# iiins0mn1a/shadow-gen

Hardware: AMD Instinct MI355X
Metric: simulated packet events/sec (whole node) at 100k hosts; APSP build time (higher is better)
Workload: dtype u64

## Files before the change

### shadow-gen_amd/csrc/engine.hip

```cpp

#include <hip/hip_runtime.h>

#include <algorithm>
#include <cstring>
#include <string>
#include <tuple>

#include "sgn_internal.h"
#include "sgn_workload.h"

#ifdef SGN_EXP_NODIGEST
#define sgn_drun_add_seq(...) ((void)0)
#define sgn_drun_add_same(...) ((void)0)
#define sgn_drun_flush_seq(...) ((void)0)
#define sgn_drun_flush_same(...) ((void)0)
#define sgn_digest3(h, ...) (h)
#endif

#ifdef SGN_DIAG
#define DG(i) ((void)0)
#define DGT_BEGIN(v) const uint64_t v = __builtin_amdgcn_s_memtime()
#define DGT_END(i, v)                                                                  \
  do {                                                                                 \
    const uint64_t dgt_t = __builtin_amdgcn_s_memtime();                               \
// ... 160 lines not shown
#ifdef SGN_EXP_PLAINCQ
  *p = e;
  return;
#endif
  SGN_GLB char* q = (SGN_GLB char*)p;
  st_wt16(q, e.enqueue_ts, e.eid);
  st_wt16(q + 16, (uint64_t)e.src | ((uint64_t)e.payload << 32), (uint64_t)e.tag | ((uint64_t)e.count << 32));
}

__device__ __forceinline__ void min_nr(SGN_GLB uint64_t* p, uint64_t v) {
  (void)__hip_atomic_fetch_min(p, v, __ATOMIC_RELAXED, __HIP_MEMORY_SCOPE_AGENT);
}

__device__ __forceinline__ void cnt_add(SGN_GLB uint64_t* p, uint64_t v) {
  (void)__hip_atomic_fetch_add(p, v, __ATOMIC_RELAXED, __HIP_MEMORY_SCOPE_AGENT);
}

__device__ __forceinline__ uint64_t div_small(uint64_t a, uint64_t b) {
  if (((a | b) >> 32) == 0) return (uint32_t)a / (uint32_t)b;
  return a / b;
}

__device__ __forceinline__ uint32_t bucket_of(const DevSim& S, uint64_t t) {
  return (uint32_t)S.bw_div.div(t - SIM_START) & (S.NB - 1);
}

__device__ __forceinline__ uint64_t codel_law(uint64_t time, uint64_t count) {
  double sq = count == 0 ? 1.0 : sqrt((double)count);
  double div = 100000000.0 / sq;
  uint64_t inc = (uint64_t)round(div);
  uint64_t orig = time - SIM_START;
  uint64_t adj = orig + inc;
  if (adj < orig || adj > SIMTIME_MAX) adj = SIMTIME_MAX;
  return SIM_START + adj;
}
// ... 617 lines not shown
    else
      fl = (fl & ~(3u << F_RI_STATE_SHIFT)) | (v << F_RI_STATE_SHIFT);
  }

  template <int W>
  __device__ __forceinline__ void forward_later(uint64_t delay) {
    set_relay_state<W>(RELAY_PENDING);
    schedule<W == 0 ? SLOT_RO : SLOT_RI>(now + delay);
  }
  template <int W>
  __device__ __forceinline__ void relay_notify() {
    if (relay_state<W>() == RELAY_IDLE) forward_later<W>(0);
  }

  template <int W>
  __device__ __forceinline__ bool tb_remove(uint64_t dec, uint64_t* dur) {
    DGT_BEGIN(tt);
    const bool ok = tb_remove_<W>(dec, dur);
    DGT_END(DGT_TBRM, tt);
    return ok;
  }
  template <int W>
  __device__ __forceinline__ bool tb_remove_(uint64_t dec, uint64_t* dur) {
    uint64_t& bal = W == 0 ? tbb0 : tbb1;
    uint64_t& last = W == 0 ? tbl0 : tbl1;
    const uint64_t interval = 1000000ULL;
    uint64_t span = now - last;
    if (span >= interval) {
      const uint64_t inc = lr().tbc[W];
      uint64_t nref = span / interval;
      uint64_t ntok = mul_sat(inc, nref, ~0ULL);
      uint64_t b = bal + ntok;
      if (b < bal) b = ~0ULL;
      const uint64_t cap = inc + SGN_CONFIG_MTU;
      bal = b > cap ? cap : b;
      uint64_t adv = mul_sat(interval, nref, SIMTIME_MAX);
      last = emu_sat_add(last, adv);
      span = now - last;
    }
    uint64_t next_refill_span = interval - span;
    if (dec > bal) {
      const uint64_t inc = lr().tbc[W];
      uint64_t req = dec - bal;
      uint64_t n;
      if (((req | inc) >> 32) == 0) {
        const uint32_t r32 = (uint32_t)req, i32 = (uint32_t)inc;
        const uint32_t q = r32 / i32;
        n = q + (r32 - q * i32 ? 1 : 0);
      } else {
        n = req / inc + ((req % inc) ? 1 : 0);
      }
      if (n == 0)
        *dur = 0;
      else if (n == 1)
        *dur = next_refill_span;
      else {
        uint64_t m = mul_sat(interval, n - 1, SIMTIME_MAX);
        uint64_t s = next_refill_span + m;
        if (s < next_refill_span || s > SIMTIME_MAX) s = SIMTIME_MAX;
        *dur = s;
      }
      return false;
    }
    bal -= dec;
    return true;
  }

  template <int K>
  __device__ __forceinline__ void dr_flush_seq() {
#ifndef SGN_EXP_NODIGEST
    const uint32_t n = L->rn[K];
    if (n) L->dig[K] = sgn_digest3(L->dig[K], L->run[K].a, L->run[K].b | ((uint64_t)n << 32), L->run[K].c - n);
    L->rn[K] = 0;
#endif
  }
  template <int K>
  __device__ __forceinline__ void dr_flush_same() {
#ifndef SGN_EXP_NODIGEST
    const uint32_t n = L->rn[K];
    if (n) L->dig[K] = sgn_digest3(L->dig[K], L->run[K].a, L->run[K].b | ((uint64_t)n << 34), L->run[K].c);
// ... 48 lines not shown
      if (I == 3) R->cq_prev = v;
    } else {
      L->cq[I] = v;
    }
  }

  __device__ __forceinline__ SGN_GLB CodelEnt* cq_head_slot() { return S.codel + cq_head; }
  __device__ __forceinline__ SGN_GLB CodelEnt* cq_tail_slot() {
    return S.codel + ((size_t)L->cq_tp * CQ_PAGE + ((cq_head + cq_nr - 1) & (CQ_PAGE - 1)));
  }
  __device__ __forceinline__ uint32_t cq_alloc_page() {
    DGT_BEGIN(ta);
    const uint64_t i = __hip_atomic_fetch_add(&C->pg_alloc, 1ULL, __ATOMIC_RELAXED, __HIP_MEMORY_SCOPE_AGENT);
    cnt_add(ob->pg_allocd, 1);
    if (i >= ob->pg_avail) return NO_HOST;
    const uint32_t pg = ld_dev(&S.cq_free[i % S.cq_pages]);
#ifdef SGN_DIAG
    DGT_WAIT();
    DGT_END(DGT_CQALLOC, ta);
#endif
    return pg;
  }
  __device__ __forceinline__ void cq_free_page(uint32_t pg) {
    DGT_BEGIN(tf);
    const uint64_t j = __hip_atomic_fetch_add(&C->pg_tail, 1ULL, __ATOMIC_RELAXED, __HIP_MEMORY_SCOPE_AGENT);
    st_dev(&S.cq_free[j % S.cq_pages], pg);
    cnt_add(ob->pg_freed, 1);
    DGT_END(DGT_CQFREE, tf);
  }
  __device__ __forceinline__ void cq_pop_head() {
    cq_nr--;
    if (cq_nr == 0) {
      cq_head &= ~(CQ_PAGE - 1);
      L->cq_tp = cq_head / CQ_PAGE;
    } else if (((cq_head + 1) & (CQ_PAGE - 1)) != 0) {
      cq_head++;
    } else {
      const uint32_t pg = cq_head / CQ_PAGE;
      const uint32_t nx = ld_dev(&S.cq_next[pg]);
      cq_free_page(pg);
      cq_head = nx * CQ_PAGE;
// ... 227 lines not shown
        p.payload = ri_pay;
        p.tag = ri_tag;
        p.eid = ri_eid;
      } else {
        if (cq_len > 0) {
          load_head();
          const bool standing = sat_sub(now, L->hd.enqueue_ts) >= CODEL_TARGET;
          const bool ie_due = (fl & F_CODEL_IE) && now >= cqg<0>();
          const bool drop_quiet = (fl & F_CODEL_DROP) && (fl & F_CODEL_DN) && now < cqg<1>();
          if (!standing || !ie_due || drop_quiet) {
            const uint32_t n = L->hd.count;
            const uint64_t wire = (uint64_t)L->hd.payload + sgn_header_bytes(L->hd.tag);
            uint32_t m = n;
            bool blocked = false;
            if (!boot) {
              if (!tb_remove<1>(wire, dur)) {
                m = 0;
                blocked = true;
              } else if (n > 1) {
                const uint64_t more = div_small(tbb1, wire);
                if (more >= n - 1) {
                  tbb1 -= (uint64_t)(n - 1) * wire;
                } else {
                  tbb1 -= more * wire;
                  m = 1 + (uint32_t)more;
                  blocked = true;
                  tb_remove<1>(wire, dur);
                }
              }
            }
            const uint32_t used = m + (blocked ? 1u : 0u);
            const CodelEnt r = L->hd;
            L->hd.eid += used;
            L->hd.count -= used;
            cq_len -= used;
            cq_bytes = sat_sub(cq_bytes, (uint64_t)used * wire);
            if (!standing || cq_bytes <= SGN_CONFIG_MTU) {
              fl &= ~(F_CODEL_IE | F_CODEL_DROP);
            } else if (!ie_due) {
              fl &= ~F_CODEL_DROP;
              if (!(fl & F_CODEL_IE)) {
                fl |= F_CODEL_IE;
                cqs<0>(emu_sat_add(now, CODEL_INTERVAL));
              }
// ... 10 lines not shown
              ri_tag = r.tag;
              ri_eid = r.eid + m;
              set_relay_state<1>(RELAY_IDLE);
              return true;
            }
            continue;
          }
        }
        const bool gotp = codel_pop(&p);
        if (!gotp) {
          set_relay_state<1>(RELAY_IDLE);
          return false;
        }
        DG(DG_FQLOAD);
      }
      if (!boot && !tb_remove<1>((uint64_t)p.payload + sgn_header_bytes(p.tag), dur)) {
        fl |= F_RI_NEXT;
        ri_src = p.src;
        ri_pay = p.payload;
        ri_tag = p.tag;
        ri_eid = p.eid;
        set_relay_state<1>(RELAY_IDLE);
        return true;
      }
      deliver_run(p.src, p.eid, 1, p.payload, p.tag);
    }
  }

  __device__ __forceinline__ void send_batch(uint32_t dst, uint32_t payload, uint32_t tag, uint32_t n,
                                             bool pop = false) {
    DGT_BEGIN(t0);
// ... 252 lines not shown
          st_dev_rec(dstp + pos + m, r);
        else
          st_sys_rec(dstp + pos + m, r);
      } else if (owned)
        place_overflow(S, ob, sidx, pos + m, r);
      else
        spill_run(S, ob, sidx, r);
    }
  }

  __device__ __forceinline__ void forward_out_step() {
    DGT_BEGIN(tf0);
    const bool boot = now < S.boot_end;
    uint64_t dur = 0;
    bool blocked = false;
    if (fl & F_RO_NEXT) {
      fl &= ~F_RO_NEXT;
      const bool is_local = ro_dst == gid;
      if (!boot && !is_local && !tb_remove<0>((uint64_t)ro_pay + sgn_header_bytes(ro_tag), &dur)) {
        fl |= F_RO_NEXT;
        blocked = true;
      } else {
        Pkt p;
        p.src = gid;
        p.dst_ip = my_ip;
        p.payload = ro_pay;
        p.tag = ro_tag;
        p.eid = 0;
        if (is_local)
          deliver_local(p);
        else
          send_batch(ro_dst, ro_pay, ro_tag, 1);
      }
    } else if (fq_len > 0) {
      const FifoEnt e = fifo_head();
      const bool rr = S.qdisc_rr && fq_len > 1;
      const uint32_t run = (e.count == 1 || rr) ? 1u : e.count - 1;
      const uint32_t payload = e.count == 1 ? (e.pay >> 16) : (e.pay & 0xFFFFu);
      const uint64_t wire = (uint64_t)payload + sgn_header_bytes(e.tag);
      const bool is_local = e.dst == gid;
      uint32_t n_ok = run;
      if (!boot && !is_local) {
        if (!tb_remove<0>(wire, &dur)) {
          n_ok = 0;
          blocked = true;
        } else if (run > 1) {
          const uint64_t more = div_small(tbb0, wire);
          if (more >= run - 1) {
            tbb0 -= (uint64_t)(run - 1) * wire;
          } else {
            tbb0 -= more * wire;
            n_ok = 1 + (uint32_t)more;
            blocked = true;
            tb_remove<0>(wire, &dur);
          }
        }
      }
      if (is_local) {
        Pkt p;
        p.src = gid;
        p.dst_ip = my_ip;
        p.payload = payload;
        p.tag = e.tag;
        p.eid = 0;
        for (uint32_t j = 0; j < n_ok; j++) {
          if (tr()) trace_pop(gid, payload, e.tag);
          deliver_local(p);
        }
      } else {
        send_batch(e.dst, payload, e.tag, n_ok, true);
      }
      if (tr() && blocked) trace_pop(e.dst, payload, e.tag);
      const uint32_t consumed = n_ok + (blocked ? 1u : 0u);
      if (consumed == e.count) {
        fq_head = fq_head + 1 == S.fifo_cap ? 0 : fq_head + 1;
        fq_len--;
        if (fq_len == 0) fq_head = 0;
        fl &= ~F_FH_DIRTY;
      } else if (rr) {
        FifoEnt m = e;
        m.count = e.count - consumed;
        fq_head = fq_head + 1 == S.fifo_cap ? 0 : fq_head + 1;
        *fq_slot(fq_len - 1) = m;
        lr().fh_idx = NO_HOST;
        fl &= ~F_FH_DIRTY;
      } else {
        if (!(fl & F_FH_DIRTY)) fq_slot(0)->count = e.count - consumed;
        L->fh.count = e.count - consumed;
      }
// ... 296 lines not shown
struct ExecLDS {
  EvRec* lev;
  uint16_t* lb;
  uint16_t* lc;
  uint32_t* lcnt;
  uint32_t* lcur;
  void* lslot;
  uint16_t* lbs;
  OutboxHdr* ob;
  uint32_t* bmin;
  struct BigLDS* big;
  uint64_t* wacc;
};


template <bool kTrace, uint32_t kApp, bool kBig, bool kXb = false, typename AtEnd>
__device__ __forceinline__ void exec_group(const DevSim& S, uint32_t g, uint64_t ws, uint64_t we, uint32_t ks,
                           const ExecLDS& X, uint64_t* kmin_out, uint64_t* next_out,
                           AtEnd&& at_end) {
  SGN_GLB Ctrl* C = S.ctrl;
  EvRec* lev = X.lev;
  uint16_t* lb = X.lb;
  uint16_t* lc = X.lc;
  uint32_t* lcnt = X.lcnt;
  uint32_t* lcur = X.lcur;
  LaneLDS<kApp>* lslot = (LaneLDS<kApp>*)X.lslot;
  uint16_t* lbs = X.lbs;
  const uint32_t lane = threadIdx.x;
  const uint32_t gsz = 1u << S.gsh;
  const uint32_t h = (g << S.gsh) + lane;
  const bool valid = lane < gsz && h < S.nH;
  const uint32_t bs = bucket_of(S, ws), be = bucket_of(S, we - 1);
  const uint32_t nbk = ((be + S.NB - bs) & (S.NB - 1)) + 1;
  const uint32_t gbase = S.lo + (g << S.gsh);
  const uint64_t clk0 = S.stamps ? __builtin_amdgcn_s_memtime() : 0;
#ifdef SGN_DIAG
  if (S.stamps && lane < 32) S.stamps[SGN_STAMP_WORDS * (size_t)g + 48 + lane] = 0;
  __syncthreads();
#endif
  const uint64_t rt0 = S.stamps ? __builtin_amdgcn_s_memrealtime() : 0;
  const size_t ik = (size_t)ks * S.G + g;
  SGN_GLB EvRec* pk = S.pool + ik * S.CAP;

  uint64_t lmin = INVALID;
  uint32_t np = NO_HOST;
  if (valid) {
    lmin = S.nextloc[h];
    if (kApp == SGN_TRAFFIC_PERIODIC) np = S.npeer[h];
  }
  Outbox<kApp>* ob = static_cast<Outbox<kApp>*>(X.ob);
  if (lane == 0) {
    ob->n = 0;
    ob->xmin = INVALID;
    ob->hz = SIM_START + (S.bw_div.div(ws - SIM_START) + S.NB) * S.BW;
  }
// ... 285 lines not shown
            else
              place_overflow(S, ob, (uint32_t)idx, pos, r);
          }
        }
      }
      const uint64_t m = __ballot(ok && e == E - 1);
      e0 += E;
      if (!m || e0 >= S.xbk) break;
      more = on && ((m >> (q * E + E - 1)) & 1ull) && e0 + e < S.xbk;
      r = EvRec{};
      if (more) r = S.xsys ? ld_sys_rec(bp + e0) : ld_dev_rec(bp + e0);
    }
    return __ballot(slow) != 0;
  };
  for (uint32_t bi = 0; bi < nbk; bi++) {
    const uint64_t c0 = S.stamps ? __builtin_amdgcn_s_memtime() : 0;
    const uint32_t b = (bs + bi) & (S.NB - 1);
    bool last = bi == nbk - 1;
    uint64_t sub_end = last ? we : SIM_START + (S.bw_div.div(ws - SIM_START) + bi + 1) * S.BW;
    const size_t ib = (size_t)uni32(S.NB <= LDS_BSLAB ? lbs[b] : ld_dev(&S.bucket_slab[b])) * S.G + g;
    const bool pair = kApp == SGN_TRAFFIC_PERIODIC && bi == 0 && nbk == 2;
    SGN_GLB const EvRec* pb = S.pool + ib * S.CAP;
    EvRec r0{}, r1{};
    size_t ib1 = 0;
    SGN_GLB const EvRec* pb1 = nullptr;
    if (pair) {
      ib1 = (size_t)(S.NB <= LDS_BSLAB ? lbs[(b + 1) & (S.NB - 1)] : ld_dev(&S.bucket_slab[(b + 1) & (S.NB - 1)])) * S.G + g;
      pb1 = S.pool + ib1 * S.CAP;
    }
    const bool bins = kXb && bi == 0 && S.xin_bins != nullptr;
    const uint32_t bsh = S.n_ranks <= 2 ? 5u : S.n_ranks <= 4 ? 4u : 3u;
// ... 84 lines not shown
      const EvRec& r = lev[idx];
      const uint32_t d = r.dst - gbase;
      const uint32_t k = lcnt[d], a = lcur[d] - k;
      uint32_t rank = 0;
      for (uint32_t t = a; k > 1 && t < a + k; t++) {
        const EvRec& o = lev[lb[t]];
        rank += (o.time < r.time ||
                 (o.time == r.time && (o.src < r.src || (o.src == r.src && o.eid < r.eid))))
                    ? 1u : 0u;
      }
      lc[a + rank] = (uint16_t)idx;
    }
    sorted += cnt > 1 ? 1u : 0u;
    if (early && !big) ex.prefetch_route();
    __syncthreads();
    const uint64_t c1 = S.stamps ? __builtin_amdgcn_s_memtime() : 0;
#ifdef SGN_DIAG
    const bool go = valid && (cnt > 0 || (loaded ? ex.next_local_time() : lmin) < until);
    const uint64_t ta = __builtin_amdgcn_s_memtime();
    if (go && !loaded) {
      ex.load();
      asm volatile("s_waitcnt vmcnt(0) lgkmcnt(0)" ::: "memory");
      loaded = true;
    }
    const uint64_t tb = __builtin_amdgcn_s_memtime();
    if (go) ex.run(lev, lc, start, start + cnt, until);
    const uint64_t tc = __builtin_amdgcn_s_memtime();
    w_load += tb - ta;
    w_run += tc - tb;
#else
    const bool go = valid && (cnt > 0 || (loaded ? ex.next_local_time() : lmin) < until);
    if (go) {
      if (!loaded) {
        ex.load();
        loaded = true;
      }
      ex.run(lev, lc, start, start + cnt, until);
    }
#endif
    if (big && fin && !go && loaded) ex.flush_digests();
    __syncthreads();
    if (S.stamps) {
      const uint64_t c2 = __builtin_amdgcn_s_memtime();
      t_gather += c1 - c0;
      t_exec += c2 - c1;
    }
      if (fin) break;
    }
  }

  {
    const uint32_t no = min(ob->n, kObox<kApp>);
    if constexpr (kApp == SGN_TRAFFIC_PERIODIC && !kBig && !kPairOff) {
      for (uint32_t i0 = 0; i0 < no; i0 += 32) {
        const uint32_t i = i0 + (lane >> 1), half = lane & 1;
        const bool has = i < no;
        uint32_t idx = 0, pos = 0;
// ... 33 lines not shown
  *next_out = m;
  const uint64_t occd = (uint64_t)wave_sum_u32((loaded ? ex.c_runs : 0u) + pk_runs) - (uint64_t)N_all;
  at_end(kmin, m, occd);
  uint32_t n_ev = 0;
#ifdef SGN_DIAG
  const uint64_t td = __builtin_amdgcn_s_memtime();
#endif
  if (loaded) {
    ex.store(lmin, np);
    n_ev = ex.c_popped + ex.c_sent + ex.c_loss + ex.c_deliv + ex.c_localev;
  }
#ifdef SGN_DIAG
  asm volatile("s_waitcnt vmcnt(0) lgkmcnt(0)" ::: "memory");
  const uint64_t w_store = __builtin_amdgcn_s_memtime() - td;
#endif
  if (S.stamps) {
    const uint64_t clk1 = __builtin_amdgcn_s_memtime();
    uint32_t sum = n_ev, mx = n_ev;
    for (int off = 32; off > 0; off >>= 1) {
      sum += __shfl_xor(sum, off, 64);
      const uint32_t o = __shfl_xor(mx, off, 64);
      mx = o > mx ? o : mx;
    }
    const uint32_t busy = __popcll(__ballot(n_ev > 0));
    SGN_GLB uint64_t* st = S.stamps + SGN_STAMP_WORDS * (size_t)g;
    if (lane == 0) {
      st[0] = clk1 - clk0;
      st[1] = sum;
      st[2] = mx;
      st[3] = busy;
      st[4] = N_all;
      st[5] = t_gather;
      st[6] = t_exec;
      st[7] = rt0;
      st[8] = ob->n;
      st[30] = __builtin_amdgcn_s_memrealtime();
    }
#ifdef SGN_DIAG
    for (int i = 0; i < DGT_N; i++) {
      const uint32_t v = loaded ? ex.dgt[i] : 0u;
// ... 290 lines not shown
      nv = want | 1u;
    } else if (++spins > (1u << 14)) {
      nv = want | 2u;
    } else {
      __builtin_amdgcn_s_sleep(2);
      continue;
    }
    uint32_t expect = v;
    if (__hip_atomic_compare_exchange_strong(&C->res_verdict, &expect, nv, __ATOMIC_RELAXED,
                                             __ATOMIC_RELAXED, __HIP_MEMORY_SCOPE_AGENT))
      *decided = true;
  }
  return v & 3u;
}

template <uint32_t kApp, bool kBig>
__global__ __launch_bounds__(64, 2) void k_rounds(const DevSim* __restrict__ Sg, uint32_t max_rounds, uint32_t epoch,
                                                  uint32_t res_base) {
  const DevSim& S = *Sg;
  SGN_GLB Ctrl* C = S.ctrl;
  SGN_EXEC_LDS(X)
  if constexpr (kApp == SGN_TRAFFIC_PERIODIC) {
    __shared__ uint64_t wacc_[W_N];
    X.wacc = wacc_;
    if (threadIdx.x < W_N) wacc_[threadIdx.x] = 0;
  }
  const uint32_t w = blockIdx.x, P = gridDim.x;
  uint32_t gq0 = w, gq1 = S.G, gqs = P;
  if constexpr (kApp == SGN_TRAFFIC_PERIODIC) {
    const uint32_t x = w & 7u, cx = (P - x + 7u) >> 3;
    uint32_t before = 0;
    for (uint32_t y = 0; y < x; y++) before += (P - y + 7u) >> 3;
    const uint32_t s0 = (uint32_t)((uint64_t)S.G * before / P), s1 = (uint32_t)((uint64_t)S.G * (before + cx) / P);
// ... 51 lines not shown
      const uint32_t q = (r + 1) % 3;
      for (uint32_t i = threadIdx.x; i < nch; i += 64) {
        st_dev(&S.rb_min[((size_t)q * RB_CH + i) * RbLayout<kApp>::MS], (uint64_t)INVALID);
        st_dev(&S.rb_min[((size_t)q * RB_CH + i) * RbLayout<kApp>::MS + 1], (uint64_t)INVALID);
        st_dev(&S.rb_occ[((size_t)q * RB_CH + i) * RbLayout<kApp>::OS], (uint64_t)0);
      }
      for (uint32_t i = threadIdx.x; i <= nch; i += 64)
        st_dev(&S.rb_cnt[(size_t)q * RbLayout<kApp>::CB + (i == nch ? RB_CH : i) * RbLayout<kApp>::CS], 0u);
      if (threadIdx.x == 0) {
        st_dev(&S.rb_keep[q], (uint64_t)INVALID);
        st_dev(&S.rb_free[q], (uint64_t)0);
        st_dev(&S.rb_occ[3 * RB_CH * RB_OS_MAX + q], (uint64_t)0);
        st_dev(&S.rb_occ[3 * RB_CH * RB_OS_MAX + 3 + q], (uint64_t)0);
      }
    }
    SGN_GLB uint64_t* rd = S.rdbg ? S.rdbg + 3 * (size_t)(r & 127) : nullptr;
    if (rd && threadIdx.x == 0)
      __hip_atomic_fetch_min(rd, (unsigned long long)__builtin_amdgcn_s_memrealtime(),
                             __ATOMIC_RELAXED, __HIP_MEMORY_SCOPE_AGENT);
    if (threadIdx.x == 0) {
      X.ob->keepmin = &S.rb_keep[p];
      X.ob->bbase = ws;
      X.ob->pg_avail = rs.pg_avail;
      X.ob->pg_freed = &S.rb_free[p];
      X.ob->pg_allocd = &S.rb_occ[3 * RB_CH * RB_OS_MAX + p];
      X.ob->spilled = &S.rb_occ[3 * RB_CH * RB_OS_MAX + 3 + p];
    }
    uint64_t kall = INVALID, mall = INVALID, oall = 0;
    bool arrived = false;
    for (uint32_t g = gq0; g < gq1; g += gqs) {
      uint64_t kmin, m;
      const bool lastg = g + gqs >= gq1;
      exec_group<false, kApp, kBig>(S, g, ws, we, ks, X, &kmin, &m, [&](uint64_t k, uint64_t n, uint64_t od) {
        kall = k < kall ? k : kall;
        mall = n < mall ? n : mall;
        oall += od;
        if (lastg) {
          if (rd && threadIdx.x == 0)
            __hip_atomic_fetch_max(rd + 1, (unsigned long long)__builtin_amdgcn_s_memrealtime(),
                                   __ATOMIC_RELAXED, __HIP_MEMORY_SCOPE_AGENT);
          flush_bmin<kApp>(S, X);
          rb_arrive<kApp>(S, p, w, P, kall, mall, oall);
          arrived = true;
        }
      });
      __syncthreads();
    }
    if (!arrived) rb_arrive<kApp>(S, p, w, P, INVALID, INVALID, 0);
// ... 80 lines not shown
      st_dev(&C->cal_occ, rs.occ);
      if (rs.hold) {
        st_dev(&C->hold, rs.hold);
        st_dev(&C->hold_need, rs.hold_need);
      }
    }
    if (S.ctrl_mirror) {
      asm volatile("s_waitcnt vmcnt(0)" ::: "memory");
      __syncthreads();
      constexpr uint32_t NW = sizeof(Ctrl) / 8;
      for (uint32_t i = threadIdx.x; i < NW; i += 64) st_sys(&S.ctrl_mirror[i], ld_dev(&((SGN_GLB uint64_t*)C)[i]));
      asm volatile("s_waitcnt vmcnt(0)" ::: "memory");
      if (threadIdx.x == 0) st_sys(&S.ctrl_mirror[NW], (uint64_t)epoch);
    }
  }
}

constexpr uint32_t XR_MAX = 8;
#ifdef SGN_XNOFENCE
constexpr bool kXFenceRel = false, kXFenceAcq = false;
#elif defined(SGN_XACQ)
constexpr bool kXFenceRel = true, kXFenceAcq = true;
#else
constexpr bool kXFenceRel = true, kXFenceAcq = false;
#endif
#ifdef SGN_KX_NOBIG
constexpr bool kKxBig = false;
#else
constexpr bool kKxBig = true;
#endif
// ... 838 lines not shown

}


namespace {

template <bool kTrace>
const void* execute_fn_t(uint32_t kind) {
  if (kind == SGN_TRAFFIC_TGEN) return (const void*)k_execute<kTrace, SGN_TRAFFIC_TGEN>;
  if (kind == SGN_TRAFFIC_EXTERNAL) return (const void*)k_execute<kTrace, SGN_TRAFFIC_EXTERNAL>;
  return (const void*)k_execute<kTrace, SGN_TRAFFIC_PERIODIC>;
}
const void* execute_fn(uint32_t kind, bool trace) {
  return trace ? execute_fn_t<true>(kind) : execute_fn_t<false>(kind);
}
template <bool kBig>
const void* rounds_fn_t(uint32_t kind) {
  if (kind == SGN_TRAFFIC_TGEN) return (const void*)k_rounds<SGN_TRAFFIC_TGEN, kBig>;
  if (kind == SGN_TRAFFIC_EXTERNAL) return (const void*)k_rounds<SGN_TRAFFIC_EXTERNAL, kBig>;
  return (const void*)k_rounds<SGN_TRAFFIC_PERIODIC, kBig>;
}
bool rounds_big(const sgn_ctx* ctx) { return ctx->ext_slabs > 0; }
const void* rounds_fn(uint32_t kind, bool big) { return big ? rounds_fn_t<true>(kind) : rounds_fn_t<false>(kind); }
template <bool kTrace>
void launch_k_execute_t(sgn_ctx* ctx, hipStream_t st) {
  const uint32_t k = ctx->S.tkind;
  const dim3 grid(ctx->S.G), block(64);
  const size_t lds = exec_lds_bytes(ctx->S.CAP, ctx->S.agg_bmin ? ctx->S.NB : 0);
  const DevSim* d = (const DevSim*)ctx->d_S;
  if (k == SGN_TRAFFIC_TGEN)
    hipLaunchKernelGGL((k_execute<kTrace, SGN_TRAFFIC_TGEN>), grid, block, lds, st, d);
  else if (k == SGN_TRAFFIC_EXTERNAL)
// ... 3 lines not shown
}
void launch_k_execute(sgn_ctx* ctx, hipStream_t st) {
  if (ctx->S.trace_on)
    launch_k_execute_t<true>(ctx, st);
  else
    launch_k_execute_t<false>(ctx, st);
}
template <bool kBig>
void launch_k_rounds_t(sgn_ctx* ctx, uint32_t n) {
  const uint32_t k = ctx->S.tkind;
  const dim3 grid(ctx->persist_grid), block(64);
  const size_t lds = exec_lds_bytes(ctx->S.CAP, ctx->S.agg_bmin ? ctx->S.NB : 0);
  const DevSim* d = (const DevSim*)ctx->d_S;
  const uint32_t ep = ++ctx->res_epoch, base = ctx->res_base;
  ctx->res_base += ctx->persist_grid;
  if (k == SGN_TRAFFIC_TGEN)
    hipLaunchKernelGGL((k_rounds<SGN_TRAFFIC_TGEN, kBig>), grid, block, lds, ctx->stream, d, n, ep, base);
  else if (k == SGN_TRAFFIC_EXTERNAL)
    hipLaunchKernelGGL((k_rounds<SGN_TRAFFIC_EXTERNAL, kBig>), grid, block, lds, ctx->stream, d, n, ep, base);
  else
    hipLaunchKernelGGL((k_rounds<SGN_TRAFFIC_PERIODIC, kBig>), grid, block, lds, ctx->stream, d, n, ep, base);
}
uint32_t census_verdict(const sgn_ctx* ctx, uint32_t epoch) {
  const uint32_t v = ctx->h_ctrl->res_verdict;
  return (v >> 2) == (epoch & 0x3FFFFFFFu) ? (v & 3u) : 0u;
}
void launch_k_rounds(sgn_ctx* ctx, uint32_t n) {
  if (rounds_big(ctx))
    launch_k_rounds_t<true>(ctx, n);
  else
// ... 277 lines not shown
  std::vector<uint32_t> ring(P), fr;
  SGN_HIP(ctx, hipMemcpy(ring.data(), (const void*)S.cq_free, P * 4, hipMemcpyDeviceToHost));
  fr.reserve(P2);
  for (uint64_t i = c.pg_alloc; i < c.pg_tail; i++) fr.push_back(ring[i % P]);
  for (uint64_t pg = P; pg < P2; pg++) fr.push_back((uint32_t)pg);
  const uint64_t nfree = fr.size();
  fr.resize(P2, 0);
  SGN_HIP(ctx, hipMemcpy(nf, fr.data(), P2 * 4, hipMemcpyHostToDevice));
  dev_free(ctx, (void*)S.codel, P * CQ_PAGE * sizeof(CodelEnt));
  dev_free(ctx, (void*)S.cq_next, P * 4);
  dev_free(ctx, (void*)S.cq_free, P * 4);
  S.codel = (decltype(S.codel))ne;
  S.cq_next = (decltype(S.cq_next))nn;
  S.cq_free = (decltype(S.cq_free))nf;
  S.cq_pages = (uint32_t)P2;
  ctx->codel_allocs_before += c.pg_alloc;
  c.pg_alloc = 0;
  c.pg_tail = c.pg_avail = nfree;
  SGN_HIP(ctx, hipMemcpy((char*)S.ctrl + offsetof(Ctrl, pg_alloc), &c.pg_alloc, 3 * 8, hipMemcpyHostToDevice));
  ctx->codel_grows++;
  return upload_sim(ctx);
}

int grow_exchange_slot_impl(sgn_ctx* ctx) {
  DevSim& S = ctx->S;
  const uint64_t hwm = ctx->h_ctrl->xhwm;
  uint64_t ns = S.xslot;
  while (ns < 2 * hwm) ns *= 2;
  if (ns > (1ULL << 26)) return set_error(ctx, SGN_EOVERFLOW, "exchange slot above 2^26 runs per peer");
  const size_t ob = XHDR + (size_t)S.xslot, nb = XHDR + (size_t)ns, R = S.n_ranks;
// ... 507 lines not shown
  S.n_all = N;
  S.lo = ctx->lo;
  S.nH = nH;
  S.U = ctx->U;
  S.end_time = SIM_START + cfg->stop_time_ns;
  S.boot_end = SIM_START + cfg->bootstrap_end_ns;
  S.runahead_cfg = cfg->runahead_ns;
  S.dynamic = cfg->use_dynamic_runahead ? 1 : 0;
  S.fifo_cap = cfg->out_fifo_cap;
  if (cfg->interface_qdisc > SGN_QDISC_ROUND_ROBIN) return set_error(ctx, SGN_EINVAL, "unknown interface_qdisc");
  S.qdisc_rr = cfg->interface_qdisc == SGN_QDISC_ROUND_ROBIN ? 1u : 0u;
  {
    const uint64_t pages = std::max<uint64_t>((uint64_t)nH + 64, ((uint64_t)nH * cfg->codel_cap + CQ_PAGE - 1) / CQ_PAGE);
    if (pages >= (1ULL << 28)) return set_error(ctx, SGN_EINVAL, "codel_cap: CoDel page pool above 2^28 pages");
    S.cq_pages = (uint32_t)pages;
  }
  S.trace_on = ctx->trace_cap > 0;
  S.tkind = tr->kind;
  S.payload_len = tr->payload_len;
  S.unknown_permille = tr->unknown_dst_permille;
  S.req_payload = tr->req_payload;
  S.n_servers = tr->kind == SGN_TRAFFIC_TGEN ? tr->n_servers : 0;
  S.flow_seed = tr->flow_seed;
  S.period = tr->period_ns;
  S.period_jitter = tr->period_jitter_ns;
  for (int i = 0; i < 3; i++) S.file_bytes[i] = tr->file_bytes[i];

  const uint64_t min_possible = ctx->lat_min, max_lat = ctx->lat_max;
  S.min_possible = min_possible;
  S.max_lat = max_lat;
// ... 1223 lines not shown
```

### shadow-gen_amd/csrc/sgn_internal.h

```cpp
#pragma once

#include <hip/hip_runtime.h>
#include <stddef.h>
#include <stdint.h>

#include <mutex>
#include <string>
#include <unordered_map>
#include <vector>

#include "sgn.h"

namespace sgn {

#ifdef __HIP_DEVICE_COMPILE__
#define SGN_GLB __attribute__((address_space(1)))
#else
#define SGN_GLB
#endif
#ifdef __HIP_DEVICE_COMPILE__
#define SGN_CONST __attribute__((address_space(4)))
#else
#define SGN_CONST
#endif
// ... 178 lines not shown
    }
    m = pm + 1;
    shift = l;
  }
  __host__ __device__ __forceinline__ uint64_t div(uint64_t x) const {
    if (m == 0) return x >> shift;
#if defined(__HIP_DEVICE_COMPILE__)
    const uint64_t q = __umul64hi(m, x);
#else
    const uint64_t q = (uint64_t)(((unsigned __int128)m * x) >> 64);
#endif
    if (add) return (((x - q) >> 1) + q) >> shift;
    return q >> shift;
  }
};

struct DevSim {
  uint32_t n_all, lo, nH, U;
  uint64_t end_time, boot_end, runahead_cfg;
  uint64_t min_possible;
  uint64_t max_lat;
  int32_t dynamic;
  uint32_t fifo_cap;
  uint32_t cq_pages;
  uint32_t qdisc_rr;
  uint32_t pad_q;
  uint32_t trace_on;
  uint32_t tkind, payload_len, unknown_permille, req_payload;
  uint32_t n_servers;
  uint32_t diag_mode;
// ... 42 lines not shown
  SGN_GLB uint64_t* w_cnt;
  SGN_GLB uint32_t* fin_cnt;
  SGN_GLB uint64_t* fin_keep;
  SGN_GLB uint64_t* fin_next;
  SGN_GLB uint64_t* fin_occ;
  SGN_GLB uint64_t* rb_min;
  SGN_GLB uint64_t* rb_keep;
  SGN_GLB uint32_t* rb_cnt;
  SGN_GLB uint64_t* rb_occ;
  uint32_t gspec;
  uint32_t fuse_finalize;
  uint32_t agg_bmin;
  uint64_t BW;
  UDiv64 bw_div;
  UDiv64 div_n, div_1000, div_ns;
  SGN_GLB uint64_t* stamps;
  SGN_GLB uint64_t* rdbg;
  uint32_t n_ranks;
  SGN_GLB Ctrl* ctrl;
  SGN_GLB sgn_trace_rec* trace;
  uint64_t trace_cap;
  SGN_GLB sgn_drain_rec* drain;
  uint64_t drain_cap;
  SGN_GLB EvRec* xout;
  SGN_GLB uint32_t* xout_n;
  SGN_GLB EvRec* xin;
  SGN_GLB uint32_t* xin_n;
  uint32_t xslot;
  uint32_t rank;
  SGN_GLB const uint32_t* rank_lo;
// ... 249 lines not shown
```

### shadow-gen_amd/csrc/snapshot.hip

```cpp
#include <algorithm>
#include <cstring>

#include "sgn_internal.h"

using namespace sgn;

namespace {

constexpr uint32_t kScanThreads = 256, kScanPer = 8, kScanTile = kScanThreads * kScanPer;
constexpr uint32_t kWaveSlabs = 64;
constexpr uint32_t kCopyWaves = 4;

__device__ __forceinline__ uint32_t slab_runs(const uint32_t* __restrict__ slab_n, const uint64_t* __restrict__ ext,
                                              uint32_t cap, uint64_t i) {
  const uint32_t room = cap + (ext ? (uint32_t)(ext[i] >> 40) : 0u);
  return min(slab_n[i], room);
}

__device__ __forceinline__ uint64_t block_excl_scan(uint64_t v, uint64_t* sh, uint64_t* total) {
  const uint32_t t = threadIdx.x;
  sh[t] = v;
  __syncthreads();
  for (uint32_t d = 1; d < kScanThreads; d <<= 1) {
    const uint64_t a = t >= d ? sh[t - d] : 0;
// ... 402 lines not shown
    dev_free(ctx, n_pool, n_slabs * Z.CAP * sizeof(EvRec));
    dev_free(ctx, n_epool, Z.ext_total * sizeof(EvRec));
    dev_free(ctx, n_ext, n_slabs * 8);
    return set_error(ctx, SGN_ENOMEM, "device allocation failed (snapshot restore)");
  }
  ctx->ctrl_fresh = false;
  ctx->rng_held.clear();
  if (codel_re) {
    dev_free(ctx, (void*)S.codel, (size_t)S.cq_pages * CQ_PAGE * sizeof(CodelEnt));
    dev_free(ctx, (void*)S.cq_next, (size_t)S.cq_pages * 4);
    dev_free(ctx, (void*)S.cq_free, (size_t)S.cq_pages * 4);
    S.codel = (decltype(S.codel))n_codel;
    S.cq_next = (decltype(S.cq_next))n_next;
    S.cq_free = (decltype(S.cq_free))n_free;
    S.cq_pages = Z.cq_pages;
  }
  if (spill_re) {
    dev_free(ctx, (void*)S.spill, S.spill_cap * sizeof(EvRec));
    dev_free(ctx, (void*)S.spill_idx, S.spill_cap * 4);
    S.spill = (decltype(S.spill))n_spill;
    S.spill_idx = (decltype(S.spill_idx))n_sidx;
    S.spill_cap = Z.spill_cap;
  }
  if (cap_re) {
    dev_free(ctx, (void*)S.pool, n_slabs * S.CAP * sizeof(EvRec));
    S.pool = (decltype(S.pool))n_pool;
    S.CAP = Z.CAP;
  }
  if (ext_re) {
    if (S.ext_pool) dev_free(ctx, (void*)S.ext_pool, S.ext_total * sizeof(EvRec));
// ... 80 lines not shown
```

Baseline: 1.811 billion.

## Batch token-bucket takes, magic-divide CoDel page ring, split diag kernel variant

Replaces the token-bucket remove-then-divide sequence with a single tb_take that computes how many packets in a run conform using 32-bit or double-based quotients. The cached relay-out path is merged into the FIFO path. CoDel free-page ring indexing switches from 64-bit modulo to a precomputed magic divider. The rounds kernel is templated on a diag flag so the stamps and rdbg instrumentation compile out of the default kernel, with a separate diag kernel used when stamps are enabled. These target 64-bit division cost and register pressure in the hot event loop, at the risk of subtle token-bucket rounding differences.

New measurement: 1.846 billion (median of 6 runs). 1.02x the previous value.

```diff
diff --git a/shadow-gen_amd/csrc/engine.hip b/shadow-gen_amd/csrc/engine.hip
--- a/shadow-gen_amd/csrc/engine.hip
+++ b/shadow-gen_amd/csrc/engine.hip
@@ -198,11 +198,6 @@
 
 __device__ __forceinline__ void cnt_add(SGN_GLB uint64_t* p, uint64_t v) {
   (void)__hip_atomic_fetch_add(p, v, __ATOMIC_RELAXED, __HIP_MEMORY_SCOPE_AGENT);
-}
-
-__device__ __forceinline__ uint64_t div_small(uint64_t a, uint64_t b) {
-  if (((a | b) >> 32) == 0) return (uint32_t)a / (uint32_t)b;
-  return a / b;
 }
 
 __device__ __forceinline__ uint32_t bucket_of(const DevSim& S, uint64_t t) {
@@ -850,14 +845,14 @@
   }
 
   template <int W>
-  __device__ __forceinline__ bool tb_remove(uint64_t dec, uint64_t* dur) {
+  __device__ __forceinline__ uint32_t tb_take(uint64_t dec, uint32_t n, uint64_t* dur) {
     DGT_BEGIN(tt);
-    const bool ok = tb_remove_<W>(dec, dur);
+    const uint32_t m = tb_take_<W>(dec, n, dur);
     DGT_END(DGT_TBRM, tt);
-    return ok;
+    return m;
   }
   template <int W>
-  __device__ __forceinline__ bool tb_remove_(uint64_t dec, uint64_t* dur) {
+  __device__ __forceinline__ uint32_t tb_take_(uint64_t dec, uint32_t n, uint64_t* dur) {
     uint64_t& bal = W == 0 ? tbb0 : tbb1;
     uint64_t& last = W == 0 ? tbl0 : tbl1;
     const uint64_t interval = 1000000ULL;
@@ -874,32 +869,21 @@
       last = emu_sat_add(last, adv);
       span = now - last;
     }
-    uint64_t next_refill_span = interval - span;
-    if (dec > bal) {
-      const uint64_t inc = lr().tbc[W];
-      uint64_t req = dec - bal;
-      uint64_t n;
-      if (((req | inc) >> 32) == 0) {
-        const uint32_t r32 = (uint32_t)req, i32 = (uint32_t)inc;
-        const uint32_t q = r32 / i32;
-        n = q + (r32 - q * i32 ? 1 : 0);
-      } else {
-        n = req / inc + ((req % inc) ? 1 : 0);
-      }
-      if (n == 0)
-        *dur = 0;
-      else if (n == 1)
+    const uint32_t m = tb_conforming(bal, dec, n);
+    bal -= (uint64_t)m * dec;
+    if (m < n) {
+      const uint64_t next_refill_span = interval - span;
+      const uint64_t nr = tb_refills(dec - bal, lr().tbc[W]);
+      if (nr == 1)
         *dur = next_refill_span;
       else {
-        uint64_t m = mul_sat(interval, n - 1, SIMTIME_MAX);
-        uint64_t s = next_refill_span + m;
+        uint64_t a = mul_sat(interval, nr - 1, SIMTIME_MAX);
+        uint64_t s = next_refill_span + a;
         if (s < next_refill_span || s > SIMTIME_MAX) s = SIMTIME_MAX;
         *dur = s;
       }
-      return false;
-    }
-    bal -= dec;
-    return true;
+    }
+    return m;
   }
 
   template <int K>
@@ -978,7 +962,7 @@
     const uint64_t i = __hip_atomic_fetch_add(&C->pg_alloc, 1ULL, __ATOMIC_RELAXED, __HIP_MEMORY_SCOPE_AGENT);
     cnt_add(ob->pg_allocd, 1);
     if (i >= ob->pg_avail) return NO_HOST;
-    const uint32_t pg = ld_dev(&S.cq_free[i % S.cq_pages]);
+    const uint32_t pg = ld_dev(&S.cq_free[umod64(S.div_cq, i, S.cq_pages)]);
 #ifdef SGN_DIAG
     DGT_WAIT();
     DGT_END(DGT_CQALLOC, ta);
@@ -988,7 +972,7 @@
   __device__ __forceinline__ void cq_free_page(uint32_t pg) {
     DGT_BEGIN(tf);
     const uint64_t j = __hip_atomic_fetch_add(&C->pg_tail, 1ULL, __ATOMIC_RELAXED, __HIP_MEMORY_SCOPE_AGENT);
-    st_dev(&S.cq_free[j % S.cq_pages], pg);
+    st_dev(&S.cq_free[umod64(S.div_cq, j, S.cq_pages)], pg);
     cnt_add(ob->pg_freed, 1);
     DGT_END(DGT_CQFREE, tf);
   }
@@ -1246,20 +1230,8 @@
             uint32_t m = n;
             bool blocked = false;
             if (!boot) {
-              if (!tb_remove<1>(wire, dur)) {
-                m = 0;
-                blocked = true;
-              } else if (n > 1) {
-                const uint64_t more = div_small(tbb1, wire);
-                if (more >= n - 1) {
-                  tbb1 -= (uint64_t)(n - 1) * wire;
-                } else {
-                  tbb1 -= more * wire;
-                  m = 1 + (uint32_t)more;
-                  blocked = true;
-                  tb_remove<1>(wire, dur);
-                }
-              }
+              m = tb_take<1>(wire, n, dur);
+              blocked = m < n;
             }
             const uint32_t used = m + (blocked ? 1u : 0u);
             const CodelEnt r = L->hd;
@@ -1300,7 +1272,7 @@
         }
         DG(DG_FQLOAD);
       }
-      if (!boot && !tb_remove<1>((uint64_t)p.payload + sgn_header_bytes(p.tag), dur)) {
+      if (!boot && tb_take<1>((uint64_t)p.payload + sgn_header_bytes(p.tag), 1, dur) == 0) {
         fl |= F_RI_NEXT;
         ri_src = p.src;
         ri_pay = p.payload;
@@ -1583,47 +1555,29 @@
     const bool boot = now < S.boot_end;
     uint64_t dur = 0;
     bool blocked = false;
-    if (fl & F_RO_NEXT) {
-      fl &= ~F_RO_NEXT;
-      const bool is_local = ro_dst == gid;
-      if (!boot && !is_local && !tb_remove<0>((uint64_t)ro_pay + sgn_header_bytes(ro_tag), &dur)) {
-        fl |= F_RO_NEXT;
-        blocked = true;
+    const bool cached = (fl & F_RO_NEXT) != 0;
+    if (cached || fq_len > 0) {
+      FifoEnt e;
+      bool rr = false;
+      uint32_t run = 1, payload;
+      if (cached) {
+        fl &= ~F_RO_NEXT;
+        e.dst = ro_dst;
+        e.tag = ro_tag;
+        e.count = 1;
+        payload = ro_pay;
       } else {
-        Pkt p;
-        p.src = gid;
-        p.dst_ip = my_ip;
-        p.payload = ro_pay;
-        p.tag = ro_tag;
-        p.eid = 0;
-        if (is_local)
-          deliver_local(p);
-        else
-          send_batch(ro_dst, ro_pay, ro_tag, 1);
-      }
-    } else if (fq_len > 0) {
-      const FifoEnt e = fifo_head();
-      const bool rr = S.qdisc_rr && fq_len > 1;
-      const uint32_t run = (e.count == 1 || rr) ? 1u : e.count - 1;
-      const uint32_t payload = e.count == 1 ? (e.pay >> 16) : (e.pay & 0xFFFFu);
+        e = fifo_head();
+        rr = S.qdisc_rr && fq_len > 1;
+        run = (e.count == 1 || rr) ? 1u : e.count - 1;
+        payload = e.count == 1 ? (e.pay >> 16) : (e.pay & 0xFFFFu);
+      }
       const uint64_t wire = (uint64_t)payload + sgn_header_bytes(e.tag);
       const bool is_local = e.dst == gid;
       uint32_t n_ok = run;
       if (!boot && !is_local) {
-        if (!tb_remove<0>(wire, &dur)) {
-          n_ok = 0;
-          blocked = true;
-        } else if (run > 1) {
-          const uint64_t more = div_small(tbb0, wire);
-          if (more >= run - 1) {
-            tbb0 -= (uint64_t)(run - 1) * wire;
-          } else {
-            tbb0 -= more * wire;
-            n_ok = 1 + (uint32_t)more;
-            blocked = true;
-            tb_remove<0>(wire, &dur);
-          }
-        }
+        n_ok = tb_take<0>(wire, run, &dur);
+        blocked = n_ok < run;
       }
       if (is_local) {
         Pkt p;
@@ -1633,15 +1587,16 @@
         p.tag = e.tag;
         p.eid = 0;
         for (uint32_t j = 0; j < n_ok; j++) {
-          if (tr()) trace_pop(gid, payload, e.tag);
+          if (tr() && !cached) trace_pop(gid, payload, e.tag);
           deliver_local(p);
         }
       } else {
-        send_batch(e.dst, payload, e.tag, n_ok, true);
-      }
-      if (tr() && blocked) trace_pop(e.dst, payload, e.tag);
+        send_batch(e.dst, payload, e.tag, n_ok, !cached);
+      }
+      if (tr() && blocked && !cached) trace_pop(e.dst, payload, e.tag);
       const uint32_t consumed = n_ok + (blocked ? 1u : 0u);
-      if (consumed == e.count) {
+      if (cached) {
+      } else if (consumed == e.count) {
         fq_head = fq_head + 1 == S.fifo_cap ? 0 : fq_head + 1;
         fq_len--;
         if (fq_len == 0) fq_head = 0;
@@ -1968,11 +1923,12 @@
 };
 
 
-template <bool kTrace, uint32_t kApp, bool kBig, bool kXb = false, typename AtEnd>
+template <bool kTrace, uint32_t kApp, bool kBig, bool kXb = false, bool kDiag = true, typename AtEnd>
 __device__ __forceinline__ void exec_group(const DevSim& S, uint32_t g, uint64_t ws, uint64_t we, uint32_t ks,
                            const ExecLDS& X, uint64_t* kmin_out, uint64_t* next_out,
                            AtEnd&& at_end) {
   SGN_GLB Ctrl* C = S.ctrl;
+  SGN_GLB uint64_t* const stamps = kDiag ? S.stamps : nullptr;
   EvRec* lev = X.lev;
   uint16_t* lb = X.lb;
   uint16_t* lc = X.lc;
@@ -1987,12 +1943,12 @@
   const uint32_t bs = bucket_of(S, ws), be = bucket_of(S, we - 1);
   const uint32_t nbk = ((be + S.NB - bs) & (S.NB - 1)) + 1;
   const uint32_t gbase = S.lo + (g << S.gsh);
-  const uint64_t clk0 = S.stamps ? __builtin_amdgcn_s_memtime() : 0;
+  const uint64_t clk0 = stamps ? __builtin_amdgcn_s_memtime() : 0;
 #ifdef SGN_DIAG
-  if (S.stamps && lane < 32) S.stamps[SGN_STAMP_WORDS * (size_t)g + 48 + lane] = 0;
+  if (stamps && lane < 32) stamps[SGN_STAMP_WORDS * (size_t)g + 48 + lane] = 0;
   __syncthreads();
 #endif
-  const uint64_t rt0 = S.stamps ? __builtin_amdgcn_s_memrealtime() : 0;
+  const uint64_t rt0 = stamps ? __builtin_amdgcn_s_memrealtime() : 0;
   const size_t ik = (size_t)ks * S.G + g;
   SGN_GLB EvRec* pk = S.pool + ik * S.CAP;
 
@@ -2308,7 +2264,7 @@
     return __ballot(slow) != 0;
   };
   for (uint32_t bi = 0; bi < nbk; bi++) {
-    const uint64_t c0 = S.stamps ? __builtin_amdgcn_s_memtime() : 0;
+    const uint64_t c0 = stamps ? __builtin_amdgcn_s_memtime() : 0;
     const uint32_t b = (bs + bi) & (S.NB - 1);
     bool last = bi == nbk - 1;
     uint64_t sub_end = last ? we : SIM_START + (S.bw_div.div(ws - SIM_START) + bi + 1) * S.BW;
@@ -2423,7 +2379,7 @@
     sorted += cnt > 1 ? 1u : 0u;
     if (early && !big) ex.prefetch_route();
     __syncthreads();
-    const uint64_t c1 = S.stamps ? __builtin_amdgcn_s_memtime() : 0;
+    const uint64_t c1 = stamps ? __builtin_amdgcn_s_memtime() : 0;
 #ifdef SGN_DIAG
     const bool go = valid && (cnt > 0 || (loaded ? ex.next_local_time() : lmin) < until);
     const uint64_t ta = __builtin_amdgcn_s_memtime();
@@ -2449,7 +2405,7 @@
 #endif
     if (big && fin && !go && loaded) ex.flush_digests();
     __syncthreads();
-    if (S.stamps) {
+    if (stamps) {
       const uint64_t c2 = __builtin_amdgcn_s_memtime();
       t_gather += c1 - c0;
       t_exec += c2 - c1;
@@ -2513,7 +2469,7 @@
   asm volatile("s_waitcnt vmcnt(0) lgkmcnt(0)" ::: "memory");
   const uint64_t w_store = __builtin_amdgcn_s_memtime() - td;
 #endif
-  if (S.stamps) {
+  if (stamps) {
     const uint64_t clk1 = __builtin_amdgcn_s_memtime();
     uint32_t sum = n_ev, mx = n_ev;
     for (int off = 32; off > 0; off >>= 1) {
@@ -2522,7 +2478,7 @@
       mx = o > mx ? o : mx;
     }
     const uint32_t busy = __popcll(__ballot(n_ev > 0));
-    SGN_GLB uint64_t* st = S.stamps + SGN_STAMP_WORDS * (size_t)g;
+    SGN_GLB uint64_t* st = stamps + SGN_STAMP_WORDS * (size_t)g;
     if (lane == 0) {
       st[0] = clk1 - clk0;
       st[1] = sum;
@@ -2843,9 +2799,9 @@
   return v & 3u;
 }
 
-template <uint32_t kApp, bool kBig>
-__global__ __launch_bounds__(64, 2) void k_rounds(const DevSim* __restrict__ Sg, uint32_t max_rounds, uint32_t epoch,
-                                                  uint32_t res_base) {
+template <uint32_t kApp, bool kBig, bool kDiag>
+__device__ __forceinline__ void rounds_body(const DevSim* __restrict__ Sg, uint32_t max_rounds, uint32_t epoch,
+                                            uint32_t res_base) {
   const DevSim& S = *Sg;
   SGN_GLB Ctrl* C = S.ctrl;
   SGN_EXEC_LDS(X)
@@ -2927,7 +2883,7 @@
         st_dev(&S.rb_occ[3 * RB_CH * RB_OS_MAX + 3 + q], (uint64_t)0);
       }
     }
-    SGN_GLB uint64_t* rd = S.rdbg ? S.rdbg + 3 * (size_t)(r & 127) : nullptr;
+    SGN_GLB uint64_t* rd = kDiag && S.rdbg ? S.rdbg + 3 * (size_t)(r & 127) : nullptr;
     if (rd && threadIdx.x == 0)
       __hip_atomic_fetch_min(rd, (unsigned long long)__builtin_amdgcn_s_memrealtime(),
                              __ATOMIC_RELAXED, __HIP_MEMORY_SCOPE_AGENT);
@@ -2944,7 +2900,7 @@
     for (uint32_t g = gq0; g < gq1; g += gqs) {
       uint64_t kmin, m;
       const bool lastg = g + gqs >= gq1;
-      exec_group<false, kApp, kBig>(S, g, ws, we, ks, X, &kmin, &m, [&](uint64_t k, uint64_t n, uint64_t od) {
+      exec_group<false, kApp, kBig, false, kDiag>(S, g, ws, we, ks, X, &kmin, &m, [&](uint64_t k, uint64_t n, uint64_t od) {
         kall = k < kall ? k : kall;
         mall = n < mall ? n : mall;
         oall += od;
@@ -3055,6 +3011,17 @@
       if (threadIdx.x == 0) st_sys(&S.ctrl_mirror[NW], (uint64_t)epoch);
     }
   }
+}
+
+template <uint32_t kApp, bool kBig>
+__global__ __launch_bounds__(64, 2) void k_rounds(const DevSim* __restrict__ Sg, uint32_t max_rounds, uint32_t epoch,
+                                                  uint32_t res_base) {
+  rounds_body<kApp, kBig, false>(Sg, max_rounds, epoch, res_base);
+}
+template <uint32_t kApp, bool kBig>
+__global__ __launch_bounds__(64, 2) void k_rounds_diag(const DevSim* __restrict__ Sg, uint32_t max_rounds,
+                                                       uint32_t epoch, uint32_t res_base) {
+  rounds_body<kApp, kBig, true>(Sg, max_rounds, epoch, res_base);
 }
 
 constexpr uint32_t XR_MAX = 8;
@@ -3923,8 +3890,14 @@
 const void* execute_fn(uint32_t kind, bool trace) {
   return trace ? execute_fn_t<true>(kind) : execute_fn_t<false>(kind);
 }
+bool rounds_diag() { return getenv("SGN_STAMPS") != nullptr; }
 template <bool kBig>
 const void* rounds_fn_t(uint32_t kind) {
+  if (rounds_diag()) {
+    if (kind == SGN_TRAFFIC_TGEN) return (const void*)k_rounds_diag<SGN_TRAFFIC_TGEN, kBig>;
+    if (kind == SGN_TRAFFIC_EXTERNAL) return (const void*)k_rounds_diag<SGN_TRAFFIC_EXTERNAL, kBig>;
+    return (const void*)k_rounds_diag<SGN_TRAFFIC_PERIODIC, kBig>;
+  }
   if (kind == SGN_TRAFFIC_TGEN) return (const void*)k_rounds<SGN_TRAFFIC_TGEN, kBig>;
   if (kind == SGN_TRAFFIC_EXTERNAL) return (const void*)k_rounds<SGN_TRAFFIC_EXTERNAL, kBig>;
   return (const void*)k_rounds<SGN_TRAFFIC_PERIODIC, kBig>;
@@ -3958,6 +3931,15 @@
   const DevSim* d = (const DevSim*)ctx->d_S;
   const uint32_t ep = ++ctx->res_epoch, base = ctx->res_base;
   ctx->res_base += ctx->persist_grid;
+  if (ctx->S.stamps) {
+    if (k == SGN_TRAFFIC_TGEN)
+      hipLaunchKernelGGL((k_rounds_diag<SGN_TRAFFIC_TGEN, kBig>), grid, block, lds, ctx->stream, d, n, ep, base);
+    else if (k == SGN_TRAFFIC_EXTERNAL)
+      hipLaunchKernelGGL((k_rounds_diag<SGN_TRAFFIC_EXTERNAL, kBig>), grid, block, lds, ctx->stream, d, n, ep, base);
+    else
+      hipLaunchKernelGGL((k_rounds_diag<SGN_TRAFFIC_PERIODIC, kBig>), grid, block, lds, ctx->stream, d, n, ep, base);
+    return;
+  }
   if (k == SGN_TRAFFIC_TGEN)
     hipLaunchKernelGGL((k_rounds<SGN_TRAFFIC_TGEN, kBig>), grid, block, lds, ctx->stream, d, n, ep, base);
   else if (k == SGN_TRAFFIC_EXTERNAL)
@@ -4265,6 +4247,7 @@
   S.cq_next = (decltype(S.cq_next))nn;
   S.cq_free = (decltype(S.cq_free))nf;
   S.cq_pages = (uint32_t)P2;
+  S.div_cq.init(P2);
   ctx->codel_allocs_before += c.pg_alloc;
   c.pg_alloc = 0;
   c.pg_tail = c.pg_avail = nfree;
@@ -4802,6 +4785,7 @@
     const uint64_t pages = std::max<uint64_t>((uint64_t)nH + 64, ((uint64_t)nH * cfg->codel_cap + CQ_PAGE - 1) / CQ_PAGE);
     if (pages >= (1ULL << 28)) return set_error(ctx, SGN_EINVAL, "codel_cap: CoDel page pool above 2^28 pages");
     S.cq_pages = (uint32_t)pages;
+    S.div_cq.init(pages);
   }
   S.trace_on = ctx->trace_cap > 0;
   S.tkind = tr->kind;
diff --git a/shadow-gen_amd/csrc/sgn_internal.h b/shadow-gen_amd/csrc/sgn_internal.h
--- a/shadow-gen_amd/csrc/sgn_internal.h
+++ b/shadow-gen_amd/csrc/sgn_internal.h
@@ -216,6 +216,35 @@
     return q >> shift;
   }
 };
+
+
+__host__ __device__ __forceinline__ uint64_t umod64(const UDiv64& d, uint64_t x, uint64_t n) {
+  return x - d.div(x) * n;
+}
+
+constexpr uint64_t TB_WIRE_MAX = 65535u + 44u;
+
+__host__ __device__ __forceinline__ uint64_t tb_refills(uint64_t req, uint64_t inc) {
+  if (inc >> 32) return 1;
+  const uint32_t r32 = (uint32_t)req, i32 = (uint32_t)inc;
+  const uint32_t q = r32 / i32;
+  return (uint64_t)q + (r32 - q * i32 ? 1 : 0);
+}
+
+__host__ __device__ __forceinline__ uint64_t tb_quot(uint64_t bal, uint64_t dec) {
+  if ((bal >> 32) == 0) return (uint32_t)bal / (uint32_t)dec;
+  uint64_t q = (uint64_t)((double)bal / (double)dec);
+  if (q * dec > bal)
+    q--;
+  else if (bal - q * dec >= dec)
+    q++;
+  return q;
+}
+
+__host__ __device__ __forceinline__ uint32_t tb_conforming(uint64_t bal, uint64_t dec, uint32_t n) {
+  if (bal >= (uint64_t)n * dec) return n;
+  return (uint32_t)tb_quot(bal, dec);
+}
 
 struct DevSim {
   uint32_t n_all, lo, nH, U;
@@ -288,6 +317,7 @@
   uint64_t BW;
   UDiv64 bw_div;
   UDiv64 div_n, div_1000, div_ns;
+  UDiv64 div_cq;
   SGN_GLB uint64_t* stamps;
   SGN_GLB uint64_t* rdbg;
   uint32_t n_ranks;
diff --git a/shadow-gen_amd/csrc/snapshot.hip b/shadow-gen_amd/csrc/snapshot.hip
--- a/shadow-gen_amd/csrc/snapshot.hip
+++ b/shadow-gen_amd/csrc/snapshot.hip
@@ -440,6 +440,7 @@
     S.cq_next = (decltype(S.cq_next))n_next;
     S.cq_free = (decltype(S.cq_free))n_free;
     S.cq_pages = Z.cq_pages;
+    S.div_cq.init(Z.cq_pages);
   }
   if (spill_re) {
     dev_free(ctx, (void*)S.spill, S.spill_cap * sizeof(EvRec));
```
